# drprojects/superpoint_transformer

Hardware: AMD Instinct MI355X
Metric: Mpoints/s SPT fwd+bwd on S3DIS-scale NAG (higher is better)
Workload: dtype f32 (the reference's shipped matmul class - configs/train.yaml:60-61 `float32_matmul_precision: high` = TF32 / bf16x3 next to `precision: 32` - as bf16x3: matrix products on the bf16 pipe with split operands, attention and the backward of the fused layers and of the attention blocks' Linears hi*hi +

## Files before the change

### include/spt_hip.h

```cpp
#ifndef SPT_HIP_H
#define SPT_HIP_H

#include <stddef.h>
#include <stdint.h>

#ifdef __cplusplus
extern "C" {
#endif

typedef void* spt_stream_t;

enum spt_reduce_op {
  SPT_SUM = 0,
  SPT_MEAN = 1,
  SPT_MIN = 2,
  SPT_MAX = 3
};

typedef struct spt_gn_fwd_tables {
  const float* weight;
  const float* mean_scale;
  float eps;
  float* mean;
  float* rstd;
// ... 107 lines not shown
                          const float* mean, const float* rstd, float act_slope,
                          float* gx, float* gweight, float* gbias,
                          float* gmean_scale, void* ws, size_t ws_bytes,
                          spt_stream_t stream);
int spt_graphnorm_stats_f32(const float* x, const int64_t* batch, int64_t r, int d, int num_graphs,
                            const float* weight, const float* mean_scale, float eps, float* mean,
                            float* rstd, float* am, float* scale, void* ws, size_t ws_bytes,
                            spt_stream_t stream);
int spt_graphnorm_bwd_acc_f32(const float* x, const float* gy, const int64_t* batch,
                              int64_t r, int d, int num_graphs, const float* weight,
                              const float* bias, const float* mean_scale,
                              const float* mean, const float* rstd, float act_slope,
                              const float* gx_add, float* gx, float* gweight, float* gbias,
                              float* gmean_scale, void* ws, size_t ws_bytes,
                              spt_stream_t stream);

int spt_edge_attn_fwd_f32(const float* qkv, int64_t n, int H, int D, int Dv,
                          const int32_t* erowptr, const int32_t* eperm,
                          const int32_t* tgt_sorted, int64_t e,
                          const float* edge_attr, int F, const float* Wk,
                          const float* bk, const float* Wq, const float* bq,
                          const float* Wv, const float* bv, int scale_mode,
                          float scale_a, float* out, float* m, float* z,
                          spt_stream_t stream);
size_t spt_edge_attn_bwd_workspace_bytes(int H, int D, int Dv, int F);
int spt_attn_use_mfma(int mode);
int spt_attn_bwd_packed(int on);
int spt_attn_bwd_el_full_line(int on);
int spt_attn_bwd_el_target_order(int on);
int spt_attn_tile_record_ints(void);
// ... 275 lines not shown
                            float* gb, const float* pre_am, const float* pre_scale,
                            const float* pre_bias, const int64_t* batch, int num_graphs, int mode,
                            void* ws, size_t ws_bytes, spt_stream_t stream);
int spt_skinny_dw_supported(int K, int N);
size_t spt_skinny_dw_workspace_bytes(int K, int N);
int spt_skinny_dw_f32(const float* gy, const float* x, int64_t rows, int N, int K, float* gw,
                      float* gb, void* ws, size_t ws_bytes, spt_stream_t stream);
int spt_skinny_linear_bwd_supported(int K, int N, int num_graphs, int mode);
size_t spt_skinny_linear_bwd_workspace_bytes(int K, int N);
int spt_skinny_linear_bwd_m_f32(const float* gy, const float* x, const float* W, int64_t rows, int N,
                                int K, float* gx, float* gw, float* gb, const float* pre_am,
                                const float* pre_scale, const float* pre_bias, const int64_t* batch,
                                int num_graphs, int mode, void* ws, size_t ws_bytes,
                                spt_stream_t stream);
int spt_skinny_bwd_fused(int on);
int spt_narrow_linear_bwd_supported(int K, int N);
size_t spt_narrow_linear_bwd_workspace_bytes(int K, int N);
int spt_narrow_linear_bwd_f32(const float* gy, const float* x, const float* W, int64_t rows, int N,
                              int K, float* gx, float* gw, float* gb, void* ws, size_t ws_bytes,
                              spt_stream_t stream);

int spt_graphnorm_tables_f32(const double* total, int num_graphs, int d, const float* weight,
                             const float* mean_scale, float eps, float* mean, float* rstd,
                             float* am, float* scale, spt_stream_t stream);
int spt_graphnorm_apply_f32(const float* x, const int64_t* batch, int64_t r, int d,
                            int num_graphs, const float* am, const float* scale,
                            const float* bias, float act_slope, float* y, spt_stream_t stream);
int spt_graphnorm_bwd_stats_f32(const float* x, const float* gy, const int64_t* batch, int64_t r,
                                int d, int num_graphs, const float* am, const float* scale,
                                const float* bias, float act_slope, double* total, void* ws,
// ... 349 lines not shown
```

### superpoint_transformer_amd/_lib.py

```python
import ctypes
import os

import torch

_HERE = os.path.dirname(os.path.abspath(__file__))
LIB_PATH = os.path.join(_HERE, "lib", "libspt_hip.so")

_c = ctypes
_i64 = _c.c_int64
_int = _c.c_int
_p = _c.c_void_p
_sz = _c.c_size_t
_f32 = _c.c_float
_f64 = _c.c_double

SIGNATURES = {
    "spt_version": (_int, []),
    "spt_last_error": (_c.c_char_p, []),
    "spt_csr_build_workspace_bytes": (_sz, [_i64, _i64]),
    "spt_csr_build": (_int, [_p, _i64, _i64, _p, _p, _p, _sz, _p]),
    "spt_csr_pos_seg": (_int, [_p, _i64, _i64, _p, _p]),
    "spt_csr_gather_i64_i32": (_int, [_p, _p, _i64, _p, _p]),
    "spt_edge_csr_build_workspace_bytes": (_sz, [_i64, _i64]),
    "spt_edge_csr_build": (_int, [_p, _i64, _i64, _i64, _p, _p, _p, _p, _p, _p, _p, _p, _sz, _p]),
# ... 9 lines not shown
    "spt_fused_linear_storage_supported": (_int, [_int, _int]),
    "spt_graphnorm_bwd_stats_sparse_ex_f32": (_int, [_p, _int, _p, _p, _p, _p, _i64, _i64, _int, _int, _p, _p,
                                                     _p, _f32, _p, _p, _sz, _p]),
    "spt_segcsr_reduce_bwd_f32": (_int, [_int, _p, _p, _p, _p, _p, _i64, _i64, _int, _p, _p]),
    "spt_segcsr_sum_i64": (_int, [_p, _p, _p, _i64, _i64, _int, _p, _p]),
    "spt_gather_rows_f32": (_int, [_p, _p, _i64, _i64, _int, _p, _p]),
    "spt_graphnorm_workspace_bytes": (_sz, [_i64, _int, _int]),
    "spt_graphnorm_fwd_f32": (_int, [_p, _p, _i64, _int, _int, _p, _p, _p, _f32, _f32,
                                     _p, _p, _p, _p, _sz, _p]),
    "spt_graphnorm_bwd_f32": (_int, [_p, _p, _p, _i64, _int, _int, _p, _p, _p, _p, _p,
                                     _f32, _p, _p, _p, _p, _p, _sz, _p]),
    "spt_graphnorm_stats_f32": (_int, [_p, _p, _i64, _int, _int, _p, _p, _f32, _p, _p, _p, _p,
                                       _p, _sz, _p]),
    "spt_graphnorm_bwd_acc_f32": (_int, [_p, _p, _p, _i64, _int, _int, _p, _p, _p, _p, _p,
                                         _f32, _p, _p, _p, _p, _p, _p, _sz, _p]),
    "spt_edge_attn_fwd_f32": (_int, [_p, _i64, _int, _int, _int, _p, _p, _p, _i64, _p, _int,
                                     _p, _p, _p, _p, _p, _p, _int, _f32, _p, _p, _p, _p]),
    "spt_edge_attn_bwd_workspace_bytes": (_sz, [_int, _int, _int, _int]),
    "spt_attn_use_mfma": (_int, [_int]),
    "spt_attn_bwd_packed": (_int, [_int]),
    "spt_attn_bwd_el_full_line": (_int, [_int]),
    "spt_attn_bwd_el_target_order": (_int, [_int]),
    "spt_attn_tile_record_ints": (_int, []),
    "spt_attn_pack_tile_ids_ex": (_int, [_p, _p, _p, _p, _i64, _p, _p]),
    "spt_attn_tile_record_ints_m": (_int, [_int]),
    "spt_attn_pack_tile_ids_m": (_int, [_p, _p, _p, _p, _i64, _int, _p, _p]),
    "spt_attn_mirror_prepare": (_int, [_p, _p, _i64, _i64, _p, _p, _p]),
    "spt_attn_pack_tile_ids_mirror": (_int, [_p, _p, _p, _p, _i64, _i64, _p, _p]),
    "spt_attn_split_pack_f32": (_int, [_p, _i64, _int, _int, _p, _p]),
    "spt_attn_split_grad_f32": (_int, [_p, _i64, _int, _int, _p, _p]),
# ... 140 lines not shown
    "spt_skinny_dw_f32": (_int, [_p, _p, _i64, _int, _int, _p, _p, _p, _sz, _p]),
    "spt_skinny_linear_f32": (_int, [_p, _i64, _int, _p, _p, _int, _p, _p]),
    "spt_skinny_linear_wt_f32": (_int, [_p, _i64, _int, _p, _int, _p, _p]),
    "spt_skinny_pre_supported": (_int, [_int, _int, _int]),
    "spt_skinny_linear_pre_f32": (_int, [_p, _i64, _int, _p, _p, _int, _p, _p, _p, _p, _p, _int, _p, _p]),
    "spt_skinny_dw_pre_f32": (_int, [_p, _p, _i64, _int, _int, _p, _p, _p, _p, _p, _p, _int, _p, _sz, _p]),
    "spt_skinny_use_split_bf16": (_int, [_int]),
    "spt_skinny_linear_pre_m_f32": (_int, [_p, _i64, _int, _p, _p, _int, _p, _p, _p, _p, _p, _int, _p, _int, _p]),
    "spt_skinny_linear_wt_m_f32": (_int, [_p, _i64, _int, _p, _int, _p, _int, _p]),
    "spt_skinny_dw_pre_m_f32": (_int, [_p, _p, _i64, _int, _int, _p, _p, _p, _p, _p, _p, _int, _int, _p, _sz, _p]),
    "spt_skinny_linear_bwd_supported": (_int, [_int, _int, _int, _int]),
    "spt_skinny_linear_bwd_workspace_bytes": (_sz, [_int, _int]),
    "spt_skinny_linear_bwd_m_f32": (_int, [_p, _p, _p, _i64, _int, _int, _p, _p, _p, _p, _p, _p, _p, _int, _int,
                                           _p, _sz, _p]),
    "spt_skinny_bwd_fused": (_int, [_int]),
    "spt_index_inverse": (_int, [_p, _i64, _i64, _p, _p]),
    "spt_select_edges_workspace_bytes": (_sz, [_i64]),
    "spt_select_edges": (_int, [_p, _i64, _i64, _p, _i64, _p, _i64, _p, _p, _p, _sz, _p]),
    "spt_cluster_select_workspace_bytes": (_sz, [_i64, _i64, _i64]),
    "spt_cluster_select": (_int, [_p, _p, _i64, _p, _i64, _i64, _p, _p, _p, _p, _p, _p, _sz, _p]),
    "spt_relabel_consecutive_workspace_bytes": (_sz, [_i64]),
    "spt_relabel_consecutive": (_int, [_p, _p, _i64, _i64, _p, _p, _p, _p, _sz, _p]),
    "spt_radius_ball_workspace_bytes": (_sz, [_i64]),
    "spt_radius_ball_f32": (_int, [_p, _i64, _p, _f32, _int, _p, _i64, _p, _p, _p, _sz, _p]),
    "spt_cluster_pair_anchors_f32": (_int, [_p, _p, _p, _p, _p, _i64, _i64, _int, _int, _p, _p, _p]),
    "spt_adjacency_stats_workspace_bytes": (_sz, [_i64]),
    "spt_adjacency_stats": (_int, [_p, _p, _i64, _i64, _int, _p, _p, _p, _sz, _p]),
    "spt_adjacency_regression": (_int, [_p, _p, _p, _i64, _i64, _int, _f32, _f32, _p, _p, _sz, _p]),
    "spt_adjacency_count_workspace_bytes": (_sz, [_i64]),
    "spt_adjacency_count": (_int, [_p, _i64, _i64, _int, _p, _p, _p, _i64, _int, _p, _p, _p, _sz, _p]),
# ... 145 lines not shown
```

### superpoint_transformer_amd/csrc/graphnorm.hip

```cpp
#include <math.h>

#include "common.hpp"

namespace spt {

constexpr int GN_THREADS = 256;
constexpr int GN_MAX_BLOCKS = 1024;
#ifndef SPT_GN_UNR
#define SPT_GN_UNR 4
#endif
constexpr int GN_UNR = SPT_GN_UNR;

struct GnShape {
  int vec, lpr_log2, rpb;
};

static bool gn_shape(int d, GnShape* s) {
  s->vec = (d % 4 == 0) ? 4 : (d % 2 == 0) ? 2 : 1;
  int lanes = d / s->vec;
  int l2 = 0;
  while ((1 << l2) < lanes) ++l2;
  if (l2 > 8) return false;
  s->lpr_log2 = l2;
  s->rpb = GN_THREADS >> l2;
// ... 639 lines not shown
                     mean, rstd, weight, mean_scale);
  (void)total;
  gn_finalize_bwd_kernel<<<(d + 15) / 16, 256, 0, stream>>>(partial, p.nblocks, B, d, weight, mean_scale, mean, rstd, am, scale, c1, c2, c3, gweight, gbias, gmean_scale);
  if (r > 0) {
    if (p.sh.vec == 4)
      gn_apply_bwd_kernel<4><<<p.nblocks * 2, GN_THREADS, 0, stream>>>(x, gy, batch, r, d, p.sh.lpr_log2, am, scale, bias, act_slope, c1, c2, c3, gx, gx_add);
    else if (p.sh.vec == 2)
      gn_apply_bwd_kernel<2><<<p.nblocks * 2, GN_THREADS, 0, stream>>>(x, gy, batch, r, d, p.sh.lpr_log2, am, scale, bias, act_slope, c1, c2, c3, gx, gx_add);
    else
      gn_apply_bwd_kernel<1><<<p.nblocks * 2, GN_THREADS, 0, stream>>>(x, gy, batch, r, d, p.sh.lpr_log2, am, scale, bias, act_slope, c1, c2, c3, gx, gx_add);
  }
  SPT_CHECK_LAUNCH();
  return 0;
}


extern "C" int spt_graphnorm_tables_f32(const double* total, int num_graphs, int d,
                                        const float* weight, const float* mean_scale,
                                        float eps, float* mean, float* rstd, float* am,
                                        float* scale, spt_stream_t stream_) {
  hipStream_t stream = (hipStream_t)stream_;
  SPT_CHECK_ARG(num_graphs >= 1 && d >= 1, "bad shape");
  SPT_CHECK_ARG(total && weight && mean_scale && mean && rstd && am && scale, "null pointer");
  gn_fwd_tables_kernel<<<(num_graphs * d + 255) / 256, 256, 0, stream>>>(
      total, num_graphs, d, weight, mean_scale, eps, mean, rstd, am, scale);
  SPT_CHECK_LAUNCH();
  return 0;
}

extern "C" int spt_graphnorm_apply_f32(const float* x, const int64_t* batch, int64_t r, int d,
// ... 197 lines not shown
```

### superpoint_transformer_amd/csrc/skinny_linear.hip

```cpp
#include "common.hpp"

namespace spt {
namespace skinny {

typedef float f32x4 __attribute__((ext_vector_type(4)));
constexpr int TR = 16;
constexpr int WAVES = 4;
constexpr int SLAB = 64;

typedef __bf16 bf16x8 __attribute__((ext_vector_type(8)));
typedef __bf16 bf16x4 __attribute__((ext_vector_type(4)));
typedef short s16x4 __attribute__((ext_vector_type(4)));

__host__ __device__ constexpr int skinny_planes(int PR) { return PR == 6 ? 3 : (PR == 3 ? 2 : 1); }
template <int NPL>
__device__ __forceinline__ void split_planes(const float (&x)[8], bf16x8 (&p)[NPL]) {
#pragma unroll
  for (int i = 0; i < 8; ++i) {
    const __bf16 a = (__bf16)x[i];
    p[0][i] = a;
    if constexpr (NPL >= 2) {
      const float r1 = x[i] - (float)a;
      const __bf16 b = (__bf16)r1;
      p[1][i] = b;
// ... 516 lines not shown
__device__ __forceinline__ bf16x8 read_tr_operand(const __bf16* at, int ld) {
  const bf16x4 a = __builtin_amdgcn_ds_read_tr16_b64_v4bf16((lds_bf16x4*)at);
  const bf16x4 b = __builtin_amdgcn_ds_read_tr16_b64_v4bf16((lds_bf16x4*)(at + 16 * ld));
  return __builtin_shufflevector(a, b, 0, 1, 2, 3, 4, 5, 6, 7);
}
template <int NPL>
__device__ __forceinline__ void split_planes4(const float4& v, bf16x4 (&p)[NPL]) {
  const float x[4] = {v.x, v.y, v.z, v.w};
#pragma unroll
  for (int i = 0; i < 4; ++i) {
    const __bf16 a = (__bf16)x[i];
    p[0][i] = a;
    if constexpr (NPL >= 2) p[1][i] = (__bf16)(x[i] - (float)a);
  }
}
template <int NN, bool PRE, int PR>
__global__ __launch_bounds__(BF_WAVES * 64, 2 * bf_per_cu(NN)) void skinny_bwd_fused_kernel(
    const float* __restrict__ gy, const float* __restrict__ x, const float* __restrict__ W, int64_t rows,
    float* __restrict__ gx, float* __restrict__ partial, const float* __restrict__ pam,
    const float* __restrict__ psc, const float* __restrict__ pbs, const int64_t* __restrict__ batch,
    int PB) {
  constexpr int K = 64, NT = BF_WAVES * 64, LDG = NN + 16, LDX = K + 16, LDW = NN + 8;
  constexpr int NPL = skinny_planes(PR), KS = NN / 32, NBW = NN / 64;
  constexpr int VG = BF_ROWS * NN / 4 / NT, VX = BF_ROWS * K / 4 / NT;
  static_assert(NN % 64 == 0 && (PR == 1 || PR == 3), "whole 64-column slabs, a bf16 mode");
  static_assert(BF_ROWS * NN / 4 % NT == 0 && BF_ROWS * K / 4 % NT == 0, "whole float4 rounds");
  constexpr int GPL = NPL == 1 ? 2 : NPL;
  static_assert(GPL * BF_ROWS * LDG * 2 >= BF_ROWS * NN * 4, "the gb slots fit the gy planes");
  __shared__ __attribute__((aligned(16))) __bf16 g_pl[GPL * BF_ROWS * LDG];
  __shared__ __attribute__((aligned(16))) __bf16 x_pl[NPL * BF_ROWS * LDX];
  __shared__ __attribute__((aligned(16))) __bf16 w_pl[NPL * K * LDW];
  __shared__ __attribute__((aligned(16))) float ptab[PRE ? 2 * PRE_MAX + K : 4];
  const int tid = threadIdx.x;
  const int lane = tid & 63;
  const int wid = __builtin_amdgcn_readfirstlane(tid >> 6);
  const int g = lane >> 4, c = lane & 15;

  for (int q = tid; q < K * (NN / 8); q += NT) {
    const int k = q & (K - 1), n8 = q / K;
    float wv[8];
#pragma unroll
    for (int j = 0; j < 8; ++j) wv[j] = W[(size_t)(8 * n8 + j) * K + k];
    bf16x8 pl[NPL];
    split_planes<NPL>(wv, pl);
#pragma unroll
    for (int p = 0; p < NPL; ++p) *reinterpret_cast<bf16x8*>(w_pl + p * K * LDW + k * LDW + 8 * n8) = pl[p];
  }
  if constexpr (PRE) {
    for (int i = tid; i < PB * K; i += NT) {
      ptab[i] = pam[i];
      ptab[PRE_MAX + i] = psc[i];
    }
    for (int i = tid; i < K; i += NT) ptab[2 * PRE_MAX + i] = pbs[i];
  }

  const int rt = wid >> 1, nh = wid & 1;
  const int kp = wid & 1, nb0 = (wid >> 1) * NBW;
  f32x4 CW[NBW][2];
#pragma unroll
  for (int i = 0; i < NBW; ++i) CW[i][0] = CW[i][1] = (f32x4){0.f, 0.f, 0.f, 0.f};
  float4 bs[VG];
#pragma unroll
  for (int v = 0; v < VG; ++v) bs[v] = make_float4(0.f, 0.f, 0.f, 0.f);

  const int64_t ntiles = (rows + BF_ROWS - 1) / BF_ROWS;
  float4 ng[VG], nx[VX];
  int xg[VX];
  auto fetch = [&](int64_t t) {
    const int64_t gbase = t * BF_ROWS * (int64_t)NN, glim = rows * (int64_t)NN;
#pragma unroll
    for (int v = 0; v < VG; ++v) {
      const int64_t e = gbase + (int64_t)(v * NT + tid) * 4;
      ng[v] = (e < glim) ? *reinterpret_cast<const float4*>(gy + e) : make_float4(0.f, 0.f, 0.f, 0.f);
    }
#pragma unroll
    for (int v = 0; v < VX; ++v) {
      const int q = v * NT + tid;
      const int64_t row = t * BF_ROWS + q / (K / 4);
      nx[v] = (row < rows) ? *reinterpret_cast<const float4*>(x + row * K + (q & (K / 4 - 1)) * 4)
                           : make_float4(0.f, 0.f, 0.f, 0.f);
      if constexpr (PRE) xg[v] = (row < rows) ? (batch ? (int)batch[row] : 0) : -1;
    }
  };
  if ((int64_t)blockIdx.x < ntiles) fetch(blockIdx.x);
  for (int64_t t = blockIdx.x; t < ntiles; t += gridDim.x) {
    __syncthreads();
#pragma unroll
    for (int v = 0; v < VG; ++v) {
      const int q4 = (v * NT + tid) * 4, rr = q4 / NN, col = q4 - rr * NN;
      bs[v].x += ng[v].x; bs[v].y += ng[v].y; bs[v].z += ng[v].z; bs[v].w += ng[v].w;
      bf16x4 pl[NPL];
      split_planes4<NPL>(ng[v], pl);
#pragma unroll
      for (int p = 0; p < NPL; ++p) *reinterpret_cast<bf16x4*>(g_pl + p * BF_ROWS * LDG + rr * LDG + col) = pl[p];
    }
#pragma unroll
    for (int v = 0; v < VX; ++v) {
      const int q = v * NT + tid, rr = q / (K / 4), ch = q & (K / 4 - 1);
      float4 w = nx[v];
      if constexpr (PRE) {
        if (xg[v] >= 0) {
          const float4 a = *reinterpret_cast<const float4*>(ptab + xg[v] * K + ch * 4);
          const float4 sc4 = *reinterpret_cast<const float4*>(ptab + PRE_MAX + xg[v] * K + ch * 4);
          const float4 b4 = *reinterpret_cast<const float4*>(ptab + 2 * PRE_MAX + ch * 4);
          w.x = fmaf(w.x - a.x, sc4.x, b4.x); w.y = fmaf(w.y - a.y, sc4.y, b4.y);
          w.z = fmaf(w.z - a.z, sc4.z, b4.z); w.w = fmaf(w.w - a.w, sc4.w, b4.w);
        }
      }
      bf16x4 pl[NPL];
      split_planes4<NPL>(w, pl);
#pragma unroll
      for (int p = 0; p < NPL; ++p) *reinterpret_cast<bf16x4*>(x_pl + p * BF_ROWS * LDX + rr * LDX + ch * 4) = pl[p];
    }
    __syncthreads();
    if (t + gridDim.x < ntiles) fetch(t + gridDim.x);

    {
      f32x4 C[2] = {(f32x4){0.f, 0.f, 0.f, 0.f}, (f32x4){0.f, 0.f, 0.f, 0.f}};
      const __bf16* al = g_pl + (16 * rt + c) * LDG + 8 * g;
#pragma unroll
      for (int ks = 0; ks < KS; ++ks) {
        bf16x8 Ap[NPL];
#pragma unroll
        for (int p = 0; p < NPL; ++p) Ap[p] = *reinterpret_cast<const bf16x8*>(al + p * BF_ROWS * LDG + 32 * ks);
#pragma unroll
        for (int i = 0; i < 2; ++i) {
          bf16x8 Bp[NPL];
#pragma unroll
          for (int p = 0; p < NPL; ++p)
            Bp[p] = *reinterpret_cast<const bf16x8*>(w_pl + p * K * LDW + (16 * (2 * nh + i) + c) * LDW +
                                                     32 * ks + 8 * g);
          C[i] = mfma_planes<PR>(Ap, Bp, C[i]);
        }
      }
#pragma unroll
      for (int r = 0; r < 4; ++r) {
        const int64_t row = t * BF_ROWS + 16 * rt + 4 * g + r;
        if (row < rows) {
#pragma unroll
          for (int i = 0; i < 2; ++i)
            __builtin_nontemporal_store(C[i][r], gx + row * K + 16 * (2 * nh + i) + c);
        }
      }
    }

#pragma unroll
    for (int s = 0; s < BF_ROWS / 32; ++s) {
      const int r0 = 32 * s + 4 * g + ((lane >> 2) & 3), c0 = 4 * (lane & 3);
      bf16x8 Ap[NBW][NPL];
#pragma unroll
      for (int i = 0; i < NBW; ++i)
#pragma unroll
        for (int p = 0; p < NPL; ++p)
          Ap[i][p] = read_tr_operand(g_pl + p * BF_ROWS * LDG + r0 * LDG + 16 * (nb0 + i) + c0, LDG);
#pragma unroll
      for (int kk = 0; kk < 2; ++kk) {
        bf16x8 Bp[NPL];
#pragma unroll
        for (int p = 0; p < NPL; ++p)
          Bp[p] = read_tr_operand(x_pl + p * BF_ROWS * LDX + r0 * LDX + 16 * (2 * kp + kk) + c0, LDX);
#pragma unroll
        for (int i = 0; i < NBW; ++i) CW[i][kk] = mfma_planes<PR>(Ap[i], Bp, CW[i][kk]);
      }
    }
  }

  float* pw = partial + (size_t)blockIdx.x * ((size_t)NN * K + NN);
#pragma unroll
  for (int i = 0; i < NBW; ++i)
#pragma unroll
    for (int kk = 0; kk < 2; ++kk)
#pragma unroll
      for (int r = 0; r < 4; ++r)
        pw[(size_t)(16 * (nb0 + i) + 4 * g + r) * K + 16 * (2 * kp + kk) + c] = CW[i][kk][r];
  __syncthreads();
  float* slots = reinterpret_cast<float*>(g_pl);
#pragma unroll
  for (int v = 0; v < VG; ++v) *reinterpret_cast<float4*>(slots + (v * NT + tid) * 4) = bs[v];
  __syncthreads();
  if (tid < NN) {
    float v = 0.f;
    for (int rr = 0; rr < BF_ROWS; ++rr) v += slots[rr * NN + tid];
    pw[(size_t)NN * K + tid] = v;
  }
}

template <int NMAX>
__global__ __launch_bounds__(256) void narrow_linear_bwd_kernel(
    const float* __restrict__ gy, const float* __restrict__ x, const float* __restrict__ W,
    int64_t rows, int N, float* __restrict__ gx, float* __restrict__ partial, int K) {
  constexpr int RT = 16;
  const int lane = (threadIdx.x & 63) + 64 * blockIdx.y;
  const int64_t wave = (int64_t)blockIdx.x * (blockDim.x >> 6) + (threadIdx.x >> 6);
  const int64_t nwaves = (int64_t)gridDim.x * (blockDim.x >> 6);
  float w[NMAX], aw[NMAX], ab[NMAX];
#pragma unroll
  for (int n = 0; n < NMAX; ++n) {
    w[n] = (n < N) ? W[(size_t)n * K + lane] : 0.f;
    aw[n] = ab[n] = 0.f;
// ... 299 lines not shown
}

static std::atomic<int> g_bwd_fused{[] { const char* e = getenv("SPT_SKINNY_BWD_FUSED"); return (e && atoi(e) == 0) ? 0 : 1; }()};
extern "C" int spt_skinny_bwd_fused(int on) {
  const int prev = g_bwd_fused;
  if (on >= 0) g_bwd_fused = on ? 1 : 0;
  return prev;
}
extern "C" int spt_skinny_linear_bwd_supported(int K, int N, int num_graphs, int mode) {
  return K == 64 && (N == 64 || N == 192) && skinny_pr_bwd(mode) != 0 && num_graphs >= 1 &&
         num_graphs * K <= PRE_MAX;
}
extern "C" size_t spt_skinny_linear_bwd_workspace_bytes(int K, int N) {
  return (size_t)BF_BLOCKS * bf_per_cu(N) * N * (K + 1) * sizeof(float);
}
extern "C" int spt_skinny_linear_bwd_m_f32(const float* gy, const float* x, const float* W, int64_t rows,
                                           int N, int K, float* gx, float* gw, float* gb,
                                           const float* pre_am, const float* pre_scale,
                                           const float* pre_bias, const int64_t* batch, int num_graphs,
                                           int mode, void* ws, size_t ws_bytes, spt_stream_t stream_) {
  const int pr = skinny_pr_bwd(mode);
  hipStream_t stream = (hipStream_t)stream_;
  SPT_CHECK_ARG(rows >= 0, "bad shape");
  const bool pre = pre_am != nullptr;
  SPT_CHECK_ARG(spt_skinny_linear_bwd_supported(K, N, pre ? num_graphs : 1, mode),
                "(K, N) not built, the f32-exact mode or num_graphs * K too large");
  SPT_CHECK_ARG(!pre || (pre_scale && pre_bias), "pre-normalisation: incomplete tables");
  SPT_CHECK_ARG(gw && (rows == 0 || (gy && x && W && gx)), "null pointer");
  SPT_CHECK_ALIGNED(gy, 16);
  SPT_CHECK_ALIGNED(x, 16);
  SPT_CHECK_ARG(ws && ws_bytes >= spt_skinny_linear_bwd_workspace_bytes(K, N), "workspace too small");
  if (rows == 0) {
    hipMemsetAsync(gw, 0, (size_t)N * K * sizeof(float), stream);
    if (gb) hipMemsetAsync(gb, 0, (size_t)N * sizeof(float), stream);
    return 0;
  }
  int64_t bx = ceil_div(rows, (int64_t)BF_ROWS);
  if (bx > BF_BLOCKS * bf_per_cu(N)) bx = BF_BLOCKS * bf_per_cu(N);
  float* partial = (float*)ws;
#define SPT_BF(NN_, PRE_, PR_)                                                                      \
  skinny_bwd_fused_kernel<NN_, PRE_, PR_><<<(unsigned)bx, BF_WAVES * 64, 0, stream>>>(               \
      gy, x, W, rows, gx, partial, pre_am, pre_scale, pre_bias, batch, num_graphs);
#define SPT_BFS(NN_, PRE_) if (pr == 3) { SPT_BF(NN_, PRE_, 3) } else { SPT_BF(NN_, PRE_, 1) }
  if (N == 192) {
    if (pre) { SPT_BFS(192, true) } else { SPT_BFS(192, false) }
  } else {
    if (pre) { SPT_BFS(64, true) } else { SPT_BFS(64, false) }
  }
#undef SPT_BFS
#undef SPT_BF
  sum_tables_kernel<<<(N * (K + 1) + 15) / 16, 1024, 0, stream>>>(partial, (int)bx, N * (K + 1), N * K, gw, gb);
  SPT_CHECK_LAUNCH();
  return 0;
}
// ... 39 lines not shown
```

### superpoint_transformer_amd/ops.py

```python
import contextlib
import ctypes
import os

import torch

from . import _lib
from . import precision as _precision
from .csr import EdgeCSR, SegmentCSR, csr_of, edge_csr_of

_OPS = {"sum": 0, "add": 0, "mean": 1, "min": 2, "max": 3}

_TIMERS = {}
_TIMER_PREFIXES = []
_TIMER_CAP = 8192


def enable_timer(name, prefix=False):
    _TIMERS[name] = []
    if prefix and name not in _TIMER_PREFIXES:
        _TIMER_PREFIXES.append(name)


def timer_count(name):
    return len(_TIMERS.get(name) or [])
# ... 848 lines not shown
    return bool(_lib.lib.spt_skinny_bwd_fused(-1 if on is None else int(bool(on))))


def skinny_bwd_route_counts():
    return dict(_BWD_ROUTE)


def _skinny_bwd_ok(g, x, weight, num_graphs, mode):
    return bool(x.is_cuda and x.dtype == torch.float32 and g.dtype == torch.float32
                and weight.dtype == torch.float32 and x.dim() == 2 and x.shape[0] >= _SKINNY_MIN_ROWS
                and _lib.lib.spt_skinny_bwd_fused(-1)
                and _lib.lib.spt_skinny_linear_bwd_supported(x.shape[1], g.shape[1], int(num_graphs),
                                                             int(mode)))


def _skinny_bwd(g, x, weight, want_bias, mode, pre=None):
    g, x, w = _dense(g), _dense(x.detach()), _dense(weight.detach())
    rows, k = x.shape
    n = g.shape[1]
    dev = x.device
    gx = torch.empty((rows, k), dtype=torch.float32, device=dev)
    gw = torch.empty((n, k), dtype=torch.float32, device=dev)
    gb = torch.empty(n, dtype=torch.float32, device=dev) if want_bias else None
    am, sc, pb, batch, B = pre if pre is not None else (None, None, None, None, 1)
    ws = _workspace(_lib.lib.spt_skinny_linear_bwd_workspace_bytes(k, n), dev)
    with torch.cuda.device(dev):
        st = _lib.lib.spt_skinny_linear_bwd_m_f32(
            _lib.ptr(g), _lib.ptr(x), _lib.ptr(w), rows, n, k, _lib.ptr(gx), _lib.ptr(gw), _lib.ptr(gb),
            _lib.ptr(am), _lib.ptr(sc), _lib.ptr(pb), _lib.ptr(batch), int(B), int(mode), _lib.ptr(ws),
            ws.numel(), _lib.stream_ptr(dev))
    _lib.check(st, "spt_skinny_linear_bwd_m_f32")
    _BWD_ROUTE["fused"] += 1
    return gx, gw, gb


class _TallLinear(torch.autograd.Function):

    @staticmethod
    def forward(ctx, x, weight, bias):
        ctx.save_for_backward(x, weight)
# ... 137 lines not shown
        ctx.meta = (B, bias is not None)
        ctx.smode = smode
        ctx.set_materialize_grads(False)
        return y, x

    @staticmethod
    def backward(ctx, gy, gres):
        xd, batch, w, b, a, mean, rstd, am, sc, wd = ctx.saved_tensors
        B, has_bias = ctx.meta
        if gy is None:
            return gres, None, None, None, None, None, None, None, None
        rows, d = xd.shape
        n = wd.shape[0]
        dev = xd.device
        gy = _dense(gy)
        if ctx.needs_input_grad[7] and _skinny_bwd_ok(gy, xd, wd, B, ctx.smode):
            gxn, gw, gb = _skinny_bwd(gy, xd, wd, has_bias, ctx.smode, (am, sc, b, batch, B))
        else:
            _BWD_ROUTE["split"] += 1
            gxn = _input_grad(gy, wd, ctx.smode)
            gw = torch.empty((n, d), dtype=torch.float32, device=dev)
            gb = torch.empty(n, dtype=torch.float32, device=dev) if has_bias else None
            ws = _workspace(_lib.lib.spt_skinny_dw_workspace_bytes(d, n), dev)
            with torch.cuda.device(dev):
                st = _lib.lib.spt_skinny_dw_pre_m_f32(
                    _lib.ptr(gy), _lib.ptr(xd), rows, n, d, _lib.ptr(gw), _lib.ptr(gb), _lib.ptr(am),
                    _lib.ptr(sc), _lib.ptr(b), _lib.ptr(batch), B, ctx.smode, _lib.ptr(ws), ws.numel(),
                    _lib.stream_ptr(dev))
            _lib.check(st, "spt_skinny_dw_pre_m_f32")
        gx = torch.empty_like(xd)
        g_w, g_b, g_a = (torch.empty(d, dtype=torch.float32, device=dev) for _ in range(3))
        if gres is not None:
            gres = _dense(gres)
        ws = _workspace(_lib.lib.spt_graphnorm_workspace_bytes(rows, d, B), dev)
        with torch.cuda.device(dev):
            st = _lib.lib.spt_graphnorm_bwd_acc_f32(
                _lib.ptr(xd), _lib.ptr(gxn), _lib.ptr(batch), rows, d, B, _lib.ptr(w), _lib.ptr(b),
                _lib.ptr(a), _lib.ptr(mean), _lib.ptr(rstd), 1.0, _lib.ptr(gres), _lib.ptr(gx),
                _lib.ptr(g_w), _lib.ptr(g_b), _lib.ptr(g_a), _lib.ptr(ws), ws.numel(),
                _lib.stream_ptr(dev))
        _lib.check(st, "spt_graphnorm_bwd_acc_f32")
        return gx, None, None, g_w, g_b, g_a, None, gw, gb


def norm_linear_ok(x, batch, num_graphs, weight):
    if not _FUSE_PRENORM or (batch is not None and num_graphs is None):
        return False
    B = 1 if batch is None else int(num_graphs)
    return bool(x.dim() == 2 and x.is_cuda and x.dtype == torch.float32
# ... 971 lines not shown
```

Before: 392.7.

## Fold graphnorm backward statistics into fused skinny linear backward kernel

The fused pre-norm linear backward kernel now also accumulates per-graph double-precision sums of the input gradient and of its product with the centred input into per-block tables, using tile-level detection of graph boundaries. A new graphnorm backward entry point finalizes from these partial tables, skipping the separate statistics pass over x and gx. This removes one full read of two activation tensors per norm-linear layer. In exchange the kernel uses more LDS and registers and runs at lower launch-bounds occupancy, adds extra synchronisation at graph boundaries, and only supports act_slope 1.

```diff
diff --git a/include/spt_hip.h b/include/spt_hip.h
--- a/include/spt_hip.h
+++ b/include/spt_hip.h
@@ -145,6 +145,14 @@
                               const float* gx_add, float* gx, float* gweight, float* gbias,
                               float* gmean_scale, void* ws, size_t ws_bytes,
                               spt_stream_t stream);
+int spt_graphnorm_bwd_acc_from_partials_f32(const float* x, const float* gy, const int64_t* batch,
+                                            int64_t r, int d, int num_graphs, const float* weight,
+                                            const float* bias, const float* mean_scale,
+                                            const float* mean, const float* rstd, float act_slope,
+                                            const float* gx_add, float* gx, float* gweight,
+                                            float* gbias, float* gmean_scale, const double* partials,
+                                            int num_partials, void* ws, size_t ws_bytes,
+                                            spt_stream_t stream);
 
 int spt_edge_attn_fwd_f32(const float* qkv, int64_t n, int H, int D, int Dv,
                           const int32_t* erowptr, const int32_t* eperm,
@@ -450,6 +458,16 @@
                                 int num_graphs, int mode, void* ws, size_t ws_bytes,
                                 spt_stream_t stream);
 int spt_skinny_bwd_fused(int on);
+int spt_skinny_linear_bwd_stats_supported(int K, int N, int num_graphs, int mode);
+int spt_skinny_linear_bwd_stats_tables(int K, int N);
+size_t spt_skinny_linear_bwd_stats_workspace_bytes(int K, int N, int num_graphs);
+int spt_skinny_linear_bwd_stats_m_f32(const float* gy, const float* x, const float* W, int64_t rows,
+                                      int N, int K, float* gx, float* gw, float* gb,
+                                      const float* pre_am, const float* pre_scale,
+                                      const float* pre_bias, const int64_t* batch, int num_graphs,
+                                      int mode, void* ws, size_t ws_bytes, double* stats,
+                                      size_t stats_bytes, spt_stream_t stream);
+int spt_prenorm_stats_fold(int on);
 int spt_narrow_linear_bwd_supported(int K, int N);
 size_t spt_narrow_linear_bwd_workspace_bytes(int K, int N);
 int spt_narrow_linear_bwd_f32(const float* gy, const float* x, const float* W, int64_t rows, int N,
diff --git a/superpoint_transformer_amd/_lib.py b/superpoint_transformer_amd/_lib.py
--- a/superpoint_transformer_amd/_lib.py
+++ b/superpoint_transformer_amd/_lib.py
@@ -47,6 +47,8 @@
                                        _p, _sz, _p]),
     "spt_graphnorm_bwd_acc_f32": (_int, [_p, _p, _p, _i64, _int, _int, _p, _p, _p, _p, _p,
                                          _f32, _p, _p, _p, _p, _p, _p, _sz, _p]),
+    "spt_graphnorm_bwd_acc_from_partials_f32": (_int, [_p, _p, _p, _i64, _int, _int, _p, _p, _p, _p, _p,
+                                                       _f32, _p, _p, _p, _p, _p, _p, _int, _p, _sz, _p]),
     "spt_edge_attn_fwd_f32": (_int, [_p, _i64, _int, _int, _int, _p, _p, _p, _i64, _p, _int,
                                      _p, _p, _p, _p, _p, _p, _int, _f32, _p, _p, _p, _p]),
     "spt_edge_attn_bwd_workspace_bytes": (_sz, [_int, _int, _int, _int]),
@@ -217,6 +219,12 @@
     "spt_skinny_linear_bwd_m_f32": (_int, [_p, _p, _p, _i64, _int, _int, _p, _p, _p, _p, _p, _p, _p, _int, _int,
                                            _p, _sz, _p]),
     "spt_skinny_bwd_fused": (_int, [_int]),
+    "spt_skinny_linear_bwd_stats_supported": (_int, [_int, _int, _int, _int]),
+    "spt_skinny_linear_bwd_stats_tables": (_int, [_int, _int]),
+    "spt_skinny_linear_bwd_stats_workspace_bytes": (_sz, [_int, _int, _int]),
+    "spt_skinny_linear_bwd_stats_m_f32": (_int, [_p, _p, _p, _i64, _int, _int, _p, _p, _p, _p, _p, _p, _p, _int,
+                                                 _int, _p, _sz, _p, _sz, _p]),
+    "spt_prenorm_stats_fold": (_int, [_int]),
     "spt_index_inverse": (_int, [_p, _i64, _i64, _p, _p]),
     "spt_select_edges_workspace_bytes": (_sz, [_i64]),
     "spt_select_edges": (_int, [_p, _i64, _i64, _p, _i64, _p, _i64, _p, _p, _p, _sz, _p]),
diff --git a/superpoint_transformer_amd/csrc/graphnorm.hip b/superpoint_transformer_amd/csrc/graphnorm.hip
--- a/superpoint_transformer_amd/csrc/graphnorm.hip
+++ b/superpoint_transformer_amd/csrc/graphnorm.hip
@@ -677,6 +677,45 @@
   return 0;
 }
 
+extern "C" int spt_graphnorm_bwd_acc_from_partials_f32(
+    const float* x, const float* gy, const int64_t* batch, int64_t r, int d, int num_graphs,
+    const float* weight, const float* bias, const float* mean_scale, const float* mean,
+    const float* rstd, float act_slope, const float* gx_add, float* gx, float* gweight, float* gbias,
+    float* gmean_scale, const double* partials, int num_partials, void* ws, size_t ws_bytes,
+    spt_stream_t stream_) {
+  hipStream_t stream = (hipStream_t)stream_;
+  const int B = num_graphs;
+  SPT_CHECK_ARG(r >= 0 && d >= 1 && B >= 1, "bad shape");
+  SPT_CHECK_ARG(act_slope == 1.f, "partial tables carry no activation mask: act_slope must be 1");
+  SPT_CHECK_ARG(partials && num_partials >= 1, "no partial tables");
+  GnPlan p;
+  SPT_CHECK_ARG(gn_plan(r, d, B, &p), "dim > 1024 unsupported");
+  if (int e = gn_check(r, d, B, p, ws, ws_bytes)) return e;
+  SPT_CHECK_ARG(weight && bias && mean_scale && mean && rstd && gweight && gbias && gmean_scale && (r == 0 || (x && gy && gx)), "null pointer");
+  SPT_CHECK_ALIGNED(x, 4 * p.sh.vec);
+  SPT_CHECK_ALIGNED(gy, 4 * p.sh.vec);
+  SPT_CHECK_ALIGNED(gx_add, 4 * p.sh.vec);
+  SPT_CHECK_ALIGNED(gx, 4 * p.sh.vec);
+  SPT_CHECK_ALIGNED(partials, 8);
+  char* base = (char*)ws;
+  float* am = (float*)(base + p.off_am);
+  float* scale = (float*)(base + p.off_scale);
+  float* c1 = (float*)(base + p.off_c1);
+  float* c2 = (float*)(base + p.off_c2);
+  float* c3 = (float*)(base + p.off_c3);
+  gn_finalize_bwd_kernel<<<(d + 15) / 16, 256, 0, stream>>>(partials, num_partials, B, d, weight, mean_scale, mean, rstd, am, scale, c1, c2, c3, gweight, gbias, gmean_scale);
+  if (r > 0) {
+    if (p.sh.vec == 4)
+      gn_apply_bwd_kernel<4><<<p.nblocks * 2, GN_THREADS, 0, stream>>>(x, gy, batch, r, d, p.sh.lpr_log2, am, scale, bias, act_slope, c1, c2, c3, gx, gx_add);
+    else if (p.sh.vec == 2)
+      gn_apply_bwd_kernel<2><<<p.nblocks * 2, GN_THREADS, 0, stream>>>(x, gy, batch, r, d, p.sh.lpr_log2, am, scale, bias, act_slope, c1, c2, c3, gx, gx_add);
+    else
+      gn_apply_bwd_kernel<1><<<p.nblocks * 2, GN_THREADS, 0, stream>>>(x, gy, batch, r, d, p.sh.lpr_log2, am, scale, bias, act_slope, c1, c2, c3, gx, gx_add);
+  }
+  SPT_CHECK_LAUNCH();
+  return 0;
+}
+
 
 extern "C" int spt_graphnorm_tables_f32(const double* total, int num_graphs, int d,
                                         const float* weight, const float* mean_scale,
diff --git a/superpoint_transformer_amd/csrc/skinny_linear.hip b/superpoint_transformer_amd/csrc/skinny_linear.hip
--- a/superpoint_transformer_amd/csrc/skinny_linear.hip
+++ b/superpoint_transformer_amd/csrc/skinny_linear.hip
@@ -554,12 +554,15 @@
     if constexpr (NPL >= 2) p[1][i] = (__bf16)(x[i] - (float)a);
   }
 }
-template <int NN, bool PRE, int PR>
-__global__ __launch_bounds__(BF_WAVES * 64, 2 * bf_per_cu(NN)) void skinny_bwd_fused_kernel(
+constexpr int ST_VALS = 4;
+__host__ __device__ constexpr int st_tab_graphs(int NN) { return NN > 64 ? 8 : 16; }
+template <int NN, bool PRE, int PR, bool ST>
+__device__ __forceinline__ void skinny_bwd_fused_body(
     const float* __restrict__ gy, const float* __restrict__ x, const float* __restrict__ W, int64_t rows,
     float* __restrict__ gx, float* __restrict__ partial, const float* __restrict__ pam,
     const float* __restrict__ psc, const float* __restrict__ pbs, const int64_t* __restrict__ batch,
-    int PB) {
+    int PB, double* __restrict__ stats, int ntab) {
+  static_assert(!ST || PRE, "statistics: the pre-norm instances");
   constexpr int K = 64, NT = BF_WAVES * 64, LDG = NN + 16, LDX = K + 16, LDW = NN + 8;
   constexpr int NPL = skinny_planes(PR), KS = NN / 32, NBW = NN / 64;
   constexpr int VG = BF_ROWS * NN / 4 / NT, VX = BF_ROWS * K / 4 / NT;
@@ -571,10 +574,28 @@
   __shared__ __attribute__((aligned(16))) __bf16 x_pl[NPL * BF_ROWS * LDX];
   __shared__ __attribute__((aligned(16))) __bf16 w_pl[NPL * K * LDW];
   __shared__ __attribute__((aligned(16))) float ptab[PRE ? 2 * PRE_MAX + K : 4];
+  constexpr int SROW = 2 * K + 1;
+  __shared__ __attribute__((aligned(16))) double st_stage[ST ? BF_WAVES * ST_VALS * 16 : 1];
+  constexpr int LDO = K + 4;
+  __shared__ __attribute__((aligned(16))) float st_o[ST ? BF_ROWS * LDO : 4];
+  __shared__ double st_tab[ST ? st_tab_graphs(NN) * SROW : 1];
+  __shared__ int st_brow[ST ? BF_ROWS : 1];
+  __shared__ int st_flag[2];
   const int tid = threadIdx.x;
   const int lane = tid & 63;
   const int wid = __builtin_amdgcn_readfirstlane(tid >> 6);
   const int g = lane >> 4, c = lane & 15;
+  const bool tab_lds = PB <= st_tab_graphs(NN);
+  double* const own = ST ? stats + (size_t)blockIdx.x * PB * SROW : nullptr;
+  double* const tab = tab_lds ? (double*)st_tab : own;
+  if constexpr (ST) {
+    if (tid < 2) st_flag[tid] = 0;
+    if (tid < SROW) {
+      for (int b = 0; b < PB; ++b) tab[b * SROW + tid] = 0.0;
+      for (int tb = blockIdx.x + gridDim.x; tb < ntab; tb += gridDim.x)
+        for (int b = 0; b < PB; ++b) stats[((size_t)tb * PB + b) * SROW + tid] = 0.0;
+    }
+  }
 
   for (int q = tid; q < K * (NN / 8); q += NT) {
     const int k = q & (K - 1), n8 = q / K;
@@ -602,6 +623,34 @@
   float4 bs[VG];
 #pragma unroll
   for (int v = 0; v < VG; ++v) bs[v] = make_float4(0.f, 0.f, 0.f, 0.f);
+
+  double s1[2] = {0.0, 0.0}, s2[2] = {0.0, 0.0};
+  int cur = 0, it = 0, ncnt = 0;
+  auto st_flush = [&](int b) {
+    if (ncnt == 0) return;
+    double v[ST_VALS] = {s1[0], s1[1], s2[0], s2[1]};
+#pragma unroll
+    for (int j = 0; j < ST_VALS; ++j) {
+      v[j] += __shfl_xor(v[j], 16, 64);
+      v[j] += __shfl_xor(v[j], 32, 64);
+      if (g == 0) st_stage[(wid * ST_VALS + j) * 16 + c] = v[j];
+    }
+    __syncthreads();
+    if (tid < SROW && b >= 0 && b < PB) {
+      double sum = (double)ncnt;
+      if (tid < 2 * K) {
+        const int col = tid & (K - 1), w0 = col >> 5, j = 2 * (tid >> 6) + ((col >> 4) & 1);
+        sum = 0.0;
+#pragma unroll
+        for (int r = 0; r < BF_WAVES / 2; ++r) sum += st_stage[((2 * r + w0) * ST_VALS + j) * 16 + (col & 15)];
+      }
+      double* p = tab + b * SROW + tid;
+      *p = *p + sum;
+    }
+    __syncthreads();
+    s1[0] = s1[1] = s2[0] = s2[1] = 0.0;
+    ncnt = 0;
+  };
 
   const int64_t ntiles = (rows + BF_ROWS - 1) / BF_ROWS;
   float4 ng[VG], nx[VX];
@@ -623,8 +672,11 @@
     }
   };
   if ((int64_t)blockIdx.x < ntiles) fetch(blockIdx.x);
-  for (int64_t t = blockIdx.x; t < ntiles; t += gridDim.x) {
+  for (int64_t t = blockIdx.x; t < ntiles; t += gridDim.x, ++it) {
     __syncthreads();
+    if constexpr (ST) {
+      if (tid == 0) st_flag[(it & 1) ^ 1] = 0;
+    }
 #pragma unroll
     for (int v = 0; v < VG; ++v) {
       const int q4 = (v * NT + tid) * 4, rr = q4 / NN, col = q4 - rr * NN;
@@ -651,8 +703,20 @@
       split_planes4<NPL>(w, pl);
 #pragma unroll
       for (int p = 0; p < NPL; ++p) *reinterpret_cast<bf16x4*>(x_pl + p * BF_ROWS * LDX + rr * LDX + ch * 4) = pl[p];
+      if constexpr (ST) {
+        float4 o = make_float4(0.f, 0.f, 0.f, 0.f);
+        if (xg[v] >= 0) {
+          const float4 a = *reinterpret_cast<const float4*>(ptab + xg[v] * K + ch * 4);
+          o = make_float4(nx[v].x - a.x, nx[v].y - a.y, nx[v].z - a.z, nx[v].w - a.w);
+        }
+        *reinterpret_cast<float4*>(st_o + rr * LDO + ch * 4) = o;
+        if (ch == 0) st_brow[rr] = xg[v];
+        if (xg[v] >= 0 && xg[v] != cur) st_flag[it & 1] = 1;
+      }
     }
     __syncthreads();
+    bool mixed = false;
+    if constexpr (ST) mixed = __builtin_amdgcn_readfirstlane(st_flag[it & 1]) != 0;
     if (t + gridDim.x < ntiles) fetch(t + gridDim.x);
 
     {
@@ -682,6 +746,44 @@
             __builtin_nontemporal_store(C[i][r], gx + row * K + 16 * (2 * nh + i) + c);
         }
       }
+      if constexpr (ST) {
+        float ov[2][4];
+#pragma unroll
+        for (int r = 0; r < 4; ++r)
+#pragma unroll
+          for (int i = 0; i < 2; ++i) ov[i][r] = st_o[(16 * rt + 4 * g + r) * LDO + 16 * (2 * nh + i) + c];
+        auto st_add = [&](int lo, int hi) {
+#pragma unroll
+          for (int r = 0; r < 4; ++r) {
+            const int lr = 16 * rt + 4 * g + r;
+            if (lr < lo || lr >= hi) continue;
+#pragma unroll
+            for (int i = 0; i < 2; ++i) {
+              const double gd = (double)C[i][r], od = (double)ov[i][r];
+              s1[i] += gd;
+              s2[i] = __builtin_fma(gd, od, s2[i]);
+            }
+          }
+          ncnt += hi - lo;
+        };
+        const int64_t left = rows - t * BF_ROWS;
+        const int nv = left < BF_ROWS ? (int)left : BF_ROWS;
+        if (!mixed) {
+          st_add(0, nv);
+        } else {
+          st_flush(cur);
+          int r0 = 0;
+          while (r0 < nv) {
+            const int b = __builtin_amdgcn_readfirstlane(st_brow[r0]);
+            int r1 = r0 + 1;
+            while (r1 < nv && __builtin_amdgcn_readfirstlane(st_brow[r1]) == b) ++r1;
+            st_add(r0, r1);
+            st_flush(b);
+            cur = b;
+            r0 = r1;
+          }
+        }
+      }
     }
 
 #pragma unroll
@@ -705,6 +807,11 @@
     }
   }
 
+  if constexpr (ST) {
+    st_flush(cur);
+    if (tab_lds && tid < SROW)
+      for (int b = 0; b < PB; ++b) own[b * SROW + tid] = st_tab[b * SROW + tid];
+  }
   float* pw = partial + (size_t)blockIdx.x * ((size_t)NN * K + NN);
 #pragma unroll
   for (int i = 0; i < NBW; ++i)
@@ -723,6 +830,23 @@
     for (int rr = 0; rr < BF_ROWS; ++rr) v += slots[rr * NN + tid];
     pw[(size_t)NN * K + tid] = v;
   }
+}
+
+template <int NN, bool PRE, int PR>
+__global__ __launch_bounds__(BF_WAVES * 64, 2 * bf_per_cu(NN)) void skinny_bwd_fused_kernel(
+    const float* __restrict__ gy, const float* __restrict__ x, const float* __restrict__ W, int64_t rows,
+    float* __restrict__ gx, float* __restrict__ partial, const float* __restrict__ pam,
+    const float* __restrict__ psc, const float* __restrict__ pbs, const int64_t* __restrict__ batch,
+    int PB) {
+  skinny_bwd_fused_body<NN, PRE, PR, false>(gy, x, W, rows, gx, partial, pam, psc, pbs, batch, PB, nullptr, 0);
+}
+template <int NN, int PR>
+__global__ __launch_bounds__(BF_WAVES * 64, 2) void skinny_bwd_prestats_kernel(
+    const float* __restrict__ gy, const float* __restrict__ x, const float* __restrict__ W, int64_t rows,
+    float* __restrict__ gx, float* __restrict__ partial, const float* __restrict__ pam,
+    const float* __restrict__ psc, const float* __restrict__ pbs, const int64_t* __restrict__ batch,
+    int PB, double* __restrict__ stats, int ntab) {
+  skinny_bwd_fused_body<NN, true, PR, true>(gy, x, W, rows, gx, partial, pam, psc, pbs, batch, PB, stats, ntab);
 }
 
 template <int NMAX>
@@ -1052,11 +1176,53 @@
 extern "C" size_t spt_skinny_linear_bwd_workspace_bytes(int K, int N) {
   return (size_t)BF_BLOCKS * bf_per_cu(N) * N * (K + 1) * sizeof(float);
 }
+static int skinny_bwd_impl(const float* gy, const float* x, const float* W, int64_t rows, int N, int K,
+                           float* gx, float* gw, float* gb, const float* pre_am, const float* pre_scale,
+                           const float* pre_bias, const int64_t* batch, int num_graphs, int mode,
+                           void* ws, size_t ws_bytes, double* stats, spt_stream_t stream_);
 extern "C" int spt_skinny_linear_bwd_m_f32(const float* gy, const float* x, const float* W, int64_t rows,
                                            int N, int K, float* gx, float* gw, float* gb,
                                            const float* pre_am, const float* pre_scale,
                                            const float* pre_bias, const int64_t* batch, int num_graphs,
                                            int mode, void* ws, size_t ws_bytes, spt_stream_t stream_) {
+  return skinny_bwd_impl(gy, x, W, rows, N, K, gx, gw, gb, pre_am, pre_scale, pre_bias, batch, num_graphs,
+                         mode, ws, ws_bytes, nullptr, stream_);
+}
+
+static std::atomic<int> g_prenorm_stats_fold{[] { const char* e = getenv("SPT_PRENORM_STATS_FOLD"); return (e && atoi(e) == 0) ? 0 : 1; }()};
+extern "C" int spt_prenorm_stats_fold(int on) {
+  const int prev = g_prenorm_stats_fold;
+  if (on >= 0) g_prenorm_stats_fold = on ? 1 : 0;
+  return prev;
+}
+extern "C" int spt_skinny_linear_bwd_stats_supported(int K, int N, int num_graphs, int mode) {
+  return spt_skinny_linear_bwd_supported(K, N, num_graphs, mode);
+}
+extern "C" int spt_skinny_linear_bwd_stats_tables(int K, int N) { return BF_BLOCKS * bf_per_cu(N); }
+extern "C" size_t spt_skinny_linear_bwd_stats_workspace_bytes(int K, int N, int num_graphs) {
+  if (K < 1 || num_graphs < 1) return 0;
+  return (size_t)spt_skinny_linear_bwd_stats_tables(K, N) * num_graphs * (2 * K + 1) * sizeof(double);
+}
+extern "C" int spt_skinny_linear_bwd_stats_m_f32(const float* gy, const float* x, const float* W,
+                                                 int64_t rows, int N, int K, float* gx, float* gw,
+                                                 float* gb, const float* pre_am, const float* pre_scale,
+                                                 const float* pre_bias, const int64_t* batch,
+                                                 int num_graphs, int mode, void* ws, size_t ws_bytes,
+                                                 double* stats, size_t stats_bytes, spt_stream_t stream_) {
+  SPT_CHECK_ARG(pre_am && pre_scale && pre_bias, "statistics: the pre-norm tables are required");
+  SPT_CHECK_ARG(spt_skinny_linear_bwd_stats_supported(K, N, num_graphs, mode),
+                "(K, N) not built, the f32-exact mode or num_graphs * K too large");
+  SPT_CHECK_ARG(stats && stats_bytes >= spt_skinny_linear_bwd_stats_workspace_bytes(K, N, num_graphs),
+                "statistics tables too small");
+  SPT_CHECK_ALIGNED(stats, 8);
+  return skinny_bwd_impl(gy, x, W, rows, N, K, gx, gw, gb, pre_am, pre_scale, pre_bias, batch, num_graphs,
+                         mode, ws, ws_bytes, stats, stream_);
+}
+
+static int skinny_bwd_impl(const float* gy, const float* x, const float* W, int64_t rows, int N, int K,
+                           float* gx, float* gw, float* gb, const float* pre_am, const float* pre_scale,
+                           const float* pre_bias, const int64_t* batch, int num_graphs, int mode,
+                           void* ws, size_t ws_bytes, double* stats, spt_stream_t stream_) {
   const int pr = skinny_pr_bwd(mode);
   hipStream_t stream = (hipStream_t)stream_;
   SPT_CHECK_ARG(rows >= 0, "bad shape");
@@ -1071,11 +1237,27 @@
   if (rows == 0) {
     hipMemsetAsync(gw, 0, (size_t)N * K * sizeof(float), stream);
     if (gb) hipMemsetAsync(gb, 0, (size_t)N * sizeof(float), stream);
+    if (stats) hipMemsetAsync(stats, 0, spt_skinny_linear_bwd_stats_workspace_bytes(K, N, num_graphs), stream);
     return 0;
   }
   int64_t bx = ceil_div(rows, (int64_t)BF_ROWS);
   if (bx > BF_BLOCKS * bf_per_cu(N)) bx = BF_BLOCKS * bf_per_cu(N);
   float* partial = (float*)ws;
+  if (stats) {
+    const int ntab = spt_skinny_linear_bwd_stats_tables(K, N);
+#define SPT_BFST(NN_, PR_)                                                                          \
+  skinny_bwd_prestats_kernel<NN_, PR_><<<(unsigned)bx, BF_WAVES * 64, 0, stream>>>(                  \
+      gy, x, W, rows, gx, partial, pre_am, pre_scale, pre_bias, batch, num_graphs, stats, ntab);
+    if (N == 192) {
+      if (pr == 3) { SPT_BFST(192, 3) } else { SPT_BFST(192, 1) }
+    } else {
+      if (pr == 3) { SPT_BFST(64, 3) } else { SPT_BFST(64, 1) }
+    }
+#undef SPT_BFST
+    sum_tables_kernel<<<(N * (K + 1) + 15) / 16, 1024, 0, stream>>>(partial, (int)bx, N * (K + 1), N * K, gw, gb);
+    SPT_CHECK_LAUNCH();
+    return 0;
+  }
 #define SPT_BF(NN_, PRE_, PR_)                                                                      \
   skinny_bwd_fused_kernel<NN_, PRE_, PR_><<<(unsigned)bx, BF_WAVES * 64, 0, stream>>>(               \
       gy, x, W, rows, gx, partial, pre_am, pre_scale, pre_bias, batch, num_graphs);
diff --git a/superpoint_transformer_amd/ops.py b/superpoint_transformer_amd/ops.py
--- a/superpoint_transformer_amd/ops.py
+++ b/superpoint_transformer_amd/ops.py
@@ -886,7 +886,24 @@
                                                              int(mode)))
 
 
-def _skinny_bwd(g, x, weight, want_bias, mode, pre=None):
+_STATS_ROUTE = {"fold": 0, "pass": 0}
+
+
+def prenorm_stats_fold(on=None):
+    return bool(_lib.lib.spt_prenorm_stats_fold(-1 if on is None else int(bool(on))))
+
+
+def prenorm_stats_route_counts():
+    return dict(_STATS_ROUTE)
+
+
+def _prenorm_stats_fold_ok(x, g, num_graphs, mode):
+    return bool(_lib.lib.spt_prenorm_stats_fold(-1)
+                and _lib.lib.spt_skinny_linear_bwd_stats_supported(x.shape[1], g.shape[1],
+                                                                   int(num_graphs), int(mode)))
+
+
+def _skinny_bwd(g, x, weight, want_bias, mode, pre=None, stats=False):
     g, x, w = _dense(g), _dense(x.detach()), _dense(weight.detach())
     rows, k = x.shape
     n = g.shape[1]
@@ -896,6 +913,18 @@
     gb = torch.empty(n, dtype=torch.float32, device=dev) if want_bias else None
     am, sc, pb, batch, B = pre if pre is not None else (None, None, None, None, 1)
     ws = _workspace(_lib.lib.spt_skinny_linear_bwd_workspace_bytes(k, n), dev)
+    if stats:
+        ntab = _lib.lib.spt_skinny_linear_bwd_stats_tables(k, n)
+        tabs = torch.empty((ntab, int(B), 2 * k + 1), dtype=torch.float64, device=dev)
+        assert tabs.numel() * 8 == _lib.lib.spt_skinny_linear_bwd_stats_workspace_bytes(k, n, int(B))
+        with torch.cuda.device(dev):
+            st = _lib.lib.spt_skinny_linear_bwd_stats_m_f32(
+                _lib.ptr(g), _lib.ptr(x), _lib.ptr(w), rows, n, k, _lib.ptr(gx), _lib.ptr(gw), _lib.ptr(gb),
+                _lib.ptr(am), _lib.ptr(sc), _lib.ptr(pb), _lib.ptr(batch), int(B), int(mode), _lib.ptr(ws),
+                ws.numel(), _lib.ptr(tabs), tabs.numel() * 8, _lib.stream_ptr(dev))
+        _lib.check(st, "spt_skinny_linear_bwd_stats_m_f32")
+        _BWD_ROUTE["fused"] += 1
+        return gx, gw, gb, tabs
     with torch.cuda.device(dev):
         st = _lib.lib.spt_skinny_linear_bwd_m_f32(
             _lib.ptr(g), _lib.ptr(x), _lib.ptr(w), rows, n, k, _lib.ptr(gx), _lib.ptr(gw), _lib.ptr(gb),
@@ -1063,8 +1092,13 @@
         n = wd.shape[0]
         dev = xd.device
         gy = _dense(gy)
+        tabs = None
         if ctx.needs_input_grad[7] and _skinny_bwd_ok(gy, xd, wd, B, ctx.smode):
-            gxn, gw, gb = _skinny_bwd(gy, xd, wd, has_bias, ctx.smode, (am, sc, b, batch, B))
+            if _prenorm_stats_fold_ok(xd, gy, B, ctx.smode):
+                gxn, gw, gb, tabs = _skinny_bwd(gy, xd, wd, has_bias, ctx.smode, (am, sc, b, batch, B),
+                                                stats=True)
+            else:
+                gxn, gw, gb = _skinny_bwd(gy, xd, wd, has_bias, ctx.smode, (am, sc, b, batch, B))
         else:
             _BWD_ROUTE["split"] += 1
             gxn = _input_grad(gy, wd, ctx.smode)
@@ -1082,6 +1116,17 @@
         if gres is not None:
             gres = _dense(gres)
         ws = _workspace(_lib.lib.spt_graphnorm_workspace_bytes(rows, d, B), dev)
+        if tabs is not None:
+            _STATS_ROUTE["fold"] += 1
+            with torch.cuda.device(dev):
+                st = _lib.lib.spt_graphnorm_bwd_acc_from_partials_f32(
+                    _lib.ptr(xd), _lib.ptr(gxn), _lib.ptr(batch), rows, d, B, _lib.ptr(w), _lib.ptr(b),
+                    _lib.ptr(a), _lib.ptr(mean), _lib.ptr(rstd), 1.0, _lib.ptr(gres), _lib.ptr(gx),
+                    _lib.ptr(g_w), _lib.ptr(g_b), _lib.ptr(g_a), _lib.ptr(tabs), tabs.shape[0],
+                    _lib.ptr(ws), ws.numel(), _lib.stream_ptr(dev))
+            _lib.check(st, "spt_graphnorm_bwd_acc_from_partials_f32")
+            return gx, None, None, g_w, g_b, g_a, None, gw, gb
+        _STATS_ROUTE["pass"] += 1
         with torch.cuda.device(dev):
             st = _lib.lib.spt_graphnorm_bwd_acc_f32(
                 _lib.ptr(xd), _lib.ptr(gxn), _lib.ptr(batch), rows, d, B, _lib.ptr(w), _lib.ptr(b),
```

New measurement: 394.7, median of 6. Within noise of the previous version (+0.5%).
